# HilaManor/AudioEditingCode

Measured on AMD Instinct MI355X. Metric: edited-clips/sec (200-step inv+edit, 10 s@16 kHz), higher is better.
Workload: dtype f32

## Files before the change

### audioeditingcode_amd/csrc/attention.hip

```cpp
#include <mutex>
#include "aed_common.h"

typedef float f32x4 __attribute__((ext_vector_type(4)));

#include "attn_params.h"

#define KV_TILE 64
#define Q_TILE 64

template <int D>
__global__ __launch_bounds__(256) void attention_kernel(AttnParams p) {
    constexpr int KLD = D + 4;
    constexpr int VLD = KV_TILE + 4;
    constexpr int NB = D / 16;
    __shared__ __attribute__((aligned(16))) float Ks[KV_TILE * KLD];
    __shared__ __attribute__((aligned(16))) float Vt[D * VLD];
    __shared__ __attribute__((aligned(16))) float Ps[4 * 16 * VLD];

    const int tid = threadIdx.x;
    const int lane = tid & 63, wave = tid >> 6;
    const int fi = lane & 15, fh = lane >> 4;
    const int b = blockIdx.z, head = blockIdx.y;
    const int q0 = blockIdx.x * Q_TILE + wave * 16;
    const int hoff = head * D;

    const float* Q = p.q + (size_t)b * p.bsq + hoff;
    const float* K = p.k + (size_t)b * p.bsk + hoff;
    const float* V = p.v + (size_t)b * p.bsv + hoff;
    const float* bias = p.bias ? p.bias + (size_t)b * p.ld_bias : nullptr;

    float4 qf[NB];
    {
        const int qr = q0 + fi;
#pragma unroll
        for (int blk = 0; blk < NB; ++blk) {
            qf[blk] = make_float4(0.f, 0.f, 0.f, 0.f);
            if (qr < p.Nq) qf[blk] = *reinterpret_cast<const float4*>(Q + (size_t)qr * p.ldq + 16 * blk + 4 * fh);
        }
    }
    f32x4 oacc[NB];
#pragma unroll
    for (int c = 0; c < NB; ++c) oacc[c] = (f32x4){0.f, 0.f, 0.f, 0.f};
    float m_run[4], l_run[4];
#pragma unroll
    for (int r = 0; r < 4; ++r) { m_run[r] = -INFINITY; l_run[r] = 0.f; }

    float* Pw = Ps + wave * 16 * VLD;

    for (int k0 = 0; k0 < p.Nk; k0 += KV_TILE) {
        for (int idx = tid; idx < KV_TILE * (D / 4); idx += 256) {
            const int key = idx / (D / 4), c4 = idx - key * (D / 4);
            float4 v = make_float4(0.f, 0.f, 0.f, 0.f);
            if (k0 + key < p.Nk) v = *reinterpret_cast<const float4*>(K + (size_t)(k0 + key) * p.ldk + 4 * c4);
            *reinterpret_cast<float4*>(Ks + key * KLD + 4 * c4) = v;
        }
        {
            const int key = tid & 63, dg = tid >> 6;
            for (int dd = dg * 4; dd < D; dd += 16) {
                float4 v = make_float4(0.f, 0.f, 0.f, 0.f);
                if (k0 + key < p.Nk) v = *reinterpret_cast<const float4*>(V + (size_t)(k0 + key) * p.ldv + dd);
                Vt[(dd + 0) * VLD + key] = v.x;
                Vt[(dd + 1) * VLD + key] = v.y;
                Vt[(dd + 2) * VLD + key] = v.z;
                Vt[(dd + 3) * VLD + key] = v.w;
            }
        }
        __syncthreads();

        f32x4 sacc[4];
#pragma unroll
        for (int j = 0; j < 4; ++j) sacc[j] = (f32x4){0.f, 0.f, 0.f, 0.f};
#pragma unroll
        for (int blk = 0; blk < NB; ++blk) {
#pragma unroll
            for (int j = 0; j < 4; ++j) {
                const float4 kf = *reinterpret_cast<const float4*>(Ks + (16 * j + fi) * KLD + 16 * blk + 4 * fh);
                sacc[j] = __builtin_amdgcn_mfma_f32_16x16x4f32(qf[blk].x, kf.x, sacc[j], 0, 0, 0);
                sacc[j] = __builtin_amdgcn_mfma_f32_16x16x4f32(qf[blk].y, kf.y, sacc[j], 0, 0, 0);
                sacc[j] = __builtin_amdgcn_mfma_f32_16x16x4f32(qf[blk].z, kf.z, sacc[j], 0, 0, 0);
                sacc[j] = __builtin_amdgcn_mfma_f32_16x16x4f32(qf[blk].w, kf.w, sacc[j], 0, 0, 0);
            }
        }
        float tmax[4];
#pragma unroll
        for (int r = 0; r < 4; ++r) tmax[r] = -INFINITY;
#pragma unroll
        for (int j = 0; j < 4; ++j) {
            const int key = k0 + 16 * j + fi;
            const bool ok = key < p.Nk;
            const float bv = (ok && bias) ? bias[key] : 0.f;
#pragma unroll
            for (int r = 0; r < 4; ++r) {
                float s = ok ? sacc[j][r] * p.scale + bv : -INFINITY;
                sacc[j][r] = s;
                tmax[r] = fmaxf(tmax[r], s);
            }
        }
#pragma unroll
        for (int r = 0; r < 4; ++r) {
#pragma unroll
            for (int o = 8; o > 0; o >>= 1) tmax[r] = fmaxf(tmax[r], __shfl_xor(tmax[r], o, 16));
        }
        float alpha[4], rsum[4];
#pragma unroll
        for (int r = 0; r < 4; ++r) {
            const float mn = fmaxf(m_run[r], tmax[r]);
            alpha[r] = __expf(m_run[r] - mn);
            m_run[r] = mn;
            rsum[r] = 0.f;
        }
#pragma unroll
        for (int j = 0; j < 4; ++j) {
#pragma unroll
            for (int r = 0; r < 4; ++r) {
                const float pv = __expf(sacc[j][r] - m_run[r]);
                rsum[r] += pv;
                Pw[(4 * fh + r) * VLD + 16 * j + fi] = pv;
            }
        }
#pragma unroll
        for (int r = 0; r < 4; ++r) {
#pragma unroll
            for (int o = 8; o > 0; o >>= 1) rsum[r] += __shfl_xor(rsum[r], o, 16);
            l_run[r] = l_run[r] * alpha[r] + rsum[r];
        }
#pragma unroll
        for (int c = 0; c < NB; ++c)
#pragma unroll
            for (int r = 0; r < 4; ++r) oacc[c][r] *= alpha[r];

        __builtin_amdgcn_fence(__ATOMIC_ACQ_REL, "wavefront");
        __builtin_amdgcn_wave_barrier();

#pragma unroll
        for (int kb = 0; kb < 4; ++kb) {
            const float4 pf = *reinterpret_cast<const float4*>(Pw + fi * VLD + 16 * kb + 4 * fh);
#pragma unroll
            for (int c = 0; c < NB; ++c) {
                const float4 vf = *reinterpret_cast<const float4*>(Vt + (16 * c + fi) * VLD + 16 * kb + 4 * fh);
                oacc[c] = __builtin_amdgcn_mfma_f32_16x16x4f32(pf.x, vf.x, oacc[c], 0, 0, 0);
                oacc[c] = __builtin_amdgcn_mfma_f32_16x16x4f32(pf.y, vf.y, oacc[c], 0, 0, 0);
                oacc[c] = __builtin_amdgcn_mfma_f32_16x16x4f32(pf.z, vf.z, oacc[c], 0, 0, 0);
                oacc[c] = __builtin_amdgcn_mfma_f32_16x16x4f32(pf.w, vf.w, oacc[c], 0, 0, 0);
            }
        }
        __syncthreads();
    }

    float* O = p.o + (size_t)b * p.bso + hoff;
#pragma unroll
    for (int r = 0; r < 4; ++r) {
        const int qr = q0 + 4 * fh + r;
        if (qr >= p.Nq) continue;
        const float inv = 1.0f / l_run[r];
#pragma unroll
        for (int c = 0; c < NB; ++c) O[(size_t)qr * p.ldo + 16 * c + fi] = oacc[c][r] * inv;
    }
}

typedef float f32x16a __attribute__((ext_vector_type(16)));

template <int D, int KSPLIT>
__global__ __launch_bounds__(256) void attention_t_kernel(AttnParams p) {
    constexpr int DT = (D + 31) / 32;
    constexpr int KLD = D + 4;
    constexpr int VLD = 32 + 4;
    constexpr int NJ = D / 8;
    constexpr int SLAB = 32 * KLD + DT * 32 * VLD;
    constexpr int MSZ = DT * 16 + 2;
    static_assert(D % 8 == 0, "head dim");
    extern __shared__ __attribute__((aligned(16))) float smem[];
    const int tid = threadIdx.x, lane = tid & 63, wave = tid >> 6;
    const int fi = lane & 31, fh = lane >> 5;
    float* Ks = smem + wave * SLAB;
    float* Vt = Ks + 32 * KLD;

    int qt, head, b;
    {
        const unsigned nx = gridDim.x, ny = gridDim.y, nwg = nx * ny * gridDim.z;
        const unsigned orig = blockIdx.x + nx * (blockIdx.y + ny * blockIdx.z);
        const unsigned xcd = orig & 7u, q = nwg >> 3, r = nwg & 7u;
        const unsigned id = (xcd < r ? xcd * (q + 1) : r * (q + 1) + (xcd - r) * q) + (orig >> 3);
        qt = (int)(id % nx);
        head = (int)((id / nx) % ny);
        b = (int)(id / (nx * ny));
    }
    const int q0 = (KSPLIT == 1 ? qt * 128 + wave * 32 : qt * 32);
    const int hoff = head * D;
    const float* Q = p.q + (size_t)b * p.bsq + hoff;
    const float* K = p.k + (size_t)b * p.bsk + hoff;
    const float* V = p.v + (size_t)b * p.bsv + hoff;
    const float* bias = p.bias ? p.bias + (size_t)b * p.ld_bias : nullptr;

    float4 qf[NJ];
    {
        const int qr = min(q0 + fi, p.Nq - 1);
#pragma unroll
        for (int j = 0; j < NJ; ++j) {
            float4 v = *reinterpret_cast<const float4*>(Q + (size_t)qr * p.ldq + 8 * j + 4 * fh);
            qf[j] = make_float4(v.x * p.scale, v.y * p.scale, v.z * p.scale, v.w * p.scale);
        }
    }
    f32x16a oacc[DT];
#pragma unroll
    for (int c = 0; c < DT; ++c)
#pragma unroll
        for (int r = 0; r < 16; ++r) oacc[c][r] = 0.f;
    float m_run = -INFINITY, l_run = 0.f;

    constexpr int KC4 = D / 4;
    constexpr int NKL = (32 * KC4) / 64;
    float4 kreg[NKL], vreg[NKL];
    const int ntiles = (p.Nk + 31) / 32;
    auto prefetch = [&](int t) {
        const int k0 = min(t, ntiles - 1) * 32;
#pragma unroll
        for (int i = 0; i < NKL; ++i) {
            const int idx = lane + 64 * i;
            const int key = min(k0 + idx / KC4, p.Nk - 1);
            kreg[i] = *reinterpret_cast<const float4*>(K + (size_t)key * p.ldk + 4 * (idx % KC4));
        }
        const int vk = min(k0 + fi, p.Nk - 1);
#pragma unroll
        for (int i = 0; i < NKL; ++i)
            vreg[i] = *reinterpret_cast<const float4*>(V + (size_t)vk * p.ldv + 4 * (2 * i + fh));
    };
    auto stage = [&]() {
#pragma unroll
        for (int i = 0; i < NKL; ++i) {
            const int idx = lane + 64 * i;
            const float4 v = kreg[i];
            *reinterpret_cast<float4*>(Ks + (idx / KC4) * KLD + 4 * (idx % KC4)) = make_float4(v.x, v.y, v.z, v.w);
        }
#pragma unroll
        for (int i = 0; i < NKL; ++i) {
            const int dd = 4 * (2 * i + fh);
            const float4 v = vreg[i];
            Vt[(dd + 0) * VLD + fi] = v.x;
            Vt[(dd + 1) * VLD + fi] = v.y;
            Vt[(dd + 2) * VLD + fi] = v.z;
            Vt[(dd + 3) * VLD + fi] = v.w;
        }
    };
    if constexpr (DT * 32 > D) {
        for (int e = lane; e < (DT * 32 - D) * VLD; e += 64) Vt[D * VLD + e] = 0.f;
    }

    const int t_first = (KSPLIT == 1 ? 0 : wave);
    constexpr int TSTEP = (KSPLIT == 1 ? 1 : KSPLIT);
    prefetch(t_first);
    for (int t = t_first; t < ntiles; t += TSTEP) {
        stage();
        prefetch(t + TSTEP);
        asm volatile("" ::: "memory");
        __builtin_amdgcn_wave_barrier();
        f32x16a sacc;
#pragma unroll
        for (int r = 0; r < 16; ++r) sacc[r] = 0.f;
#pragma unroll
        for (int j = 0; j < NJ; ++j) {
            const float4 kf = *reinterpret_cast<const float4*>(Ks + fi * KLD + 8 * j + 4 * fh);
            sacc = __builtin_amdgcn_mfma_f32_32x32x2f32(kf.x, qf[j].x, sacc, 0, 0, 0);
            sacc = __builtin_amdgcn_mfma_f32_32x32x2f32(kf.y, qf[j].y, sacc, 0, 0, 0);
            sacc = __builtin_amdgcn_mfma_f32_32x32x2f32(kf.z, qf[j].z, sacc, 0, 0, 0);
            sacc = __builtin_amdgcn_mfma_f32_32x32x2f32(kf.w, qf[j].w, sacc, 0, 0, 0);
        }
        const int k0 = t * 32;
        if (bias) {
#pragma unroll
            for (int rq = 0; rq < 4; ++rq)
#pragma unroll
                for (int e = 0; e < 4; ++e)
                    sacc[4 * rq + e] += bias[min(k0 + 8 * rq + 4 * fh + e, p.Nk - 1)];
        }
        if (k0 + 32 > p.Nk) {
#pragma unroll
            for (int r = 0; r < 16; ++r)
                if (k0 + (r & 3) + 8 * (r >> 2) + 4 * fh >= p.Nk) sacc[r] = -INFINITY;
        }
        float mx = sacc[0];
#pragma unroll
        for (int r = 1; r < 16; ++r) mx = fmaxf(mx, sacc[r]);
        {
            auto sw = __builtin_amdgcn_permlane32_swap(__float_as_uint(mx), __float_as_uint(mx), false, false);
            mx = fmaxf(__uint_as_float(sw[0]), __uint_as_float(sw[1]));
        }
        const float mn = fmaxf(m_run, mx);
        const float alpha = __expf(m_run - mn);
        m_run = mn;
        float rsum = 0.f;
#pragma unroll
        for (int r = 0; r < 16; ++r) {
            sacc[r] = __expf(sacc[r] - mn);
            rsum += sacc[r];
        }
        l_run = l_run * alpha + rsum;
#pragma unroll
        for (int c = 0; c < DT; ++c)
#pragma unroll
            for (int r = 0; r < 16; ++r) oacc[c][r] *= alpha;
#pragma unroll
        for (int rq = 0; rq < 4; ++rq) {
#pragma unroll
            for (int c = 0; c < DT; ++c) {
                const float4 vf = *reinterpret_cast<const float4*>(Vt + (c * 32 + fi) * VLD + 8 * rq + 4 * fh);
                oacc[c] = __builtin_amdgcn_mfma_f32_32x32x2f32(vf.x, sacc[4 * rq + 0], oacc[c], 0, 0, 0);
                oacc[c] = __builtin_amdgcn_mfma_f32_32x32x2f32(vf.y, sacc[4 * rq + 1], oacc[c], 0, 0, 0);
                oacc[c] = __builtin_amdgcn_mfma_f32_32x32x2f32(vf.z, sacc[4 * rq + 2], oacc[c], 0, 0, 0);
                oacc[c] = __builtin_amdgcn_mfma_f32_32x32x2f32(vf.w, sacc[4 * rq + 3], oacc[c], 0, 0, 0);
            }
        }
        asm volatile("" ::: "memory");
        __builtin_amdgcn_wave_barrier();
    }

    if constexpr (KSPLIT > 1) {
        __syncthreads();
        float* mrg = smem;
        if (wave > 0) {
            float* dst = mrg + ((wave - 1) * 64 + lane) * MSZ;
            dst[0] = m_run;
            dst[1] = l_run;
#pragma unroll
            for (int c = 0; c < DT; ++c)
#pragma unroll
                for (int r = 0; r < 16; ++r) dst[2 + 16 * c + r] = oacc[c][r];
        }
        __syncthreads();
        if (wave > 0) return;
        float mt = m_run;
#pragma unroll
        for (int w = 0; w < KSPLIT - 1; ++w) mt = fmaxf(mt, mrg[(w * 64 + lane) * MSZ]);
        const float a0 = (m_run == -INFINITY) ? 0.f : __expf(m_run - mt);
        l_run *= a0;
#pragma unroll
        for (int c = 0; c < DT; ++c)
#pragma unroll
            for (int r = 0; r < 16; ++r) oacc[c][r] *= a0;
#pragma unroll
        for (int w = 0; w < KSPLIT - 1; ++w) {
            const float* src = mrg + (w * 64 + lane) * MSZ;
            const float mw = src[0];
            const float aw = (mw == -INFINITY) ? 0.f : __expf(mw - mt);
            l_run += src[1] * aw;
#pragma unroll
            for (int c = 0; c < DT; ++c)
#pragma unroll
                for (int r = 0; r < 16; ++r) oacc[c][r] += src[2 + 16 * c + r] * aw;
        }
    }
    {
        auto sw = __builtin_amdgcn_permlane32_swap(__float_as_uint(l_run), __float_as_uint(l_run), false, false);
        l_run = __uint_as_float(sw[0]) + __uint_as_float(sw[1]);
    }
    const float inv = 1.0f / l_run;
    const int qr = q0 + fi;
    if (qr < p.Nq) {
        float* O = p.o + (size_t)b * p.bso + hoff + (size_t)qr * p.ldo;
#pragma unroll
        for (int c = 0; c < DT; ++c)
#pragma unroll
            for (int rq = 0; rq < 4; ++rq) {
                const int d0 = c * 32 + 8 * rq + 4 * fh;
                if (d0 < D)
                    *reinterpret_cast<float4*>(O + d0) = make_float4(oacc[c][4 * rq] * inv, oacc[c][4 * rq + 1] * inv,
                                                                     oacc[c][4 * rq + 2] * inv, oacc[c][4 * rq + 3] * inv);
            }
    }
}

template <int D, int KSPLIT>
static int launch_t(const AttnParams& p, int B, hipStream_t s) {
    constexpr int DT = (D + 31) / 32;
    constexpr int SLAB = 32 * (D + 4) + DT * 32 * 36;
    constexpr int MRG = (KSPLIT - 1) * 64 * (DT * 16 + 2);
    const size_t bytes = sizeof(float) * (4 * SLAB > MRG ? 4 * SLAB : MRG);
    static std::once_flag attr_once;
    static hipError_t attr_rc = hipSuccess;
    std::call_once(attr_once, [&] {
        attr_rc = hipFuncSetAttribute((const void*)attention_t_kernel<D, KSPLIT>,
                                      hipFuncAttributeMaxDynamicSharedMemorySize, (int)bytes);
    });
    AED_CHECK_HIP(attr_rc);
    dim3 grid(aed_cdiv(p.Nq, KSPLIT == 1 ? 128 : 32), p.H, B);
    hipLaunchKernelGGL((attention_t_kernel<D, KSPLIT>), grid, dim3(256), bytes, s, p);
    return 0;
}

int launch_attention(const aed_op* op, hipStream_t s) {
    const int32_t* i = op->i;
    AttnParams p;
    p.q = (const float*)op->p[0]; p.k = (const float*)op->p[1]; p.v = (const float*)op->p[2];
    p.bias = (const float*)op->p[3]; p.o = (float*)op->p[4];
    AED_REQUIRE(p.q && p.k && p.v && p.o, "attention: null pointer");
    p.H = i[1]; p.Nq = i[2]; p.Nk = i[3];
    p.ldq = i[5]; p.ldk = i[6]; p.ldv = i[7]; p.ldo = i[8]; p.ld_bias = i[9];
    p.bsq = i[10]; p.bsk = i[11]; p.bsv = i[12]; p.bso = i[13];
    p.scale = op->f[0];
    AED_REQUIRE(p.ldq % 4 == 0 && p.ldk % 4 == 0 && p.ldv % 4 == 0, "attention: row strides must be multiples of 4");
    AED_REQUIRE(p.Nq > 0 && p.Nk > 0, "attention: empty sequence");
    AED_REQUIRE(p.ldo % 4 == 0, "attention: output row stride must be a multiple of 4");
    if (p.Nk > KV_TILE && i[14] != 1) {
        const long wg_ksplit1 = (long)aed_cdiv(p.Nq, 128) * p.H * i[0];
        const bool ks4 = wg_ksplit1 < 2L * aed_num_cus();
        int rc = 0;
        if (((op->flags & 4) && !ks4) || i[14] == 3) {
            rc = launch_attention_x6(p, i[0], i[4], s);
            if (rc >= 0) return rc;
            AED_REQUIRE(i[14] != 3, "attention: the split-bf16 kernel does not take head dim %d / these operands", i[4]);
        }
        switch (i[4]) {
            case 32: rc = ks4 ? launch_t<32, 4>(p, i[0], s) : launch_t<32, 1>(p, i[0], s); break;
            case 48: rc = ks4 ? launch_t<48, 4>(p, i[0], s) : launch_t<48, 1>(p, i[0], s); break;
            case 64: rc = ks4 ? launch_t<64, 4>(p, i[0], s) : launch_t<64, 1>(p, i[0], s); break;
            case 80: rc = ks4 ? launch_t<80, 4>(p, i[0], s) : launch_t<80, 1>(p, i[0], s); break;
            case 16: rc = ks4 ? launch_t<16, 4>(p, i[0], s) : launch_t<16, 1>(p, i[0], s); break;
            default: AED_REQUIRE(false, "attention: unsupported head dim %d (16/32/48/64/80)", i[4]);
        }
        if (rc) return rc;
        AED_CHECK_HIP(hipGetLastError());
        return 0;
    }
    dim3 grid(aed_cdiv(p.Nq, Q_TILE), p.H, i[0]);
    switch (i[4]) {
        case 16: hipLaunchKernelGGL(attention_kernel<16>, grid, dim3(256), 0, s, p); break;
        case 32: hipLaunchKernelGGL(attention_kernel<32>, grid, dim3(256), 0, s, p); break;
        case 48: hipLaunchKernelGGL(attention_kernel<48>, grid, dim3(256), 0, s, p); break;
        case 64: hipLaunchKernelGGL(attention_kernel<64>, grid, dim3(256), 0, s, p); break;
        case 80: hipLaunchKernelGGL(attention_kernel<80>, grid, dim3(256), 0, s, p); break;
        default: AED_REQUIRE(false, "attention: unsupported head dim %d (16/32/48/64/80)", i[4]);
    }
    AED_CHECK_HIP(hipGetLastError());
    return 0;
}
```

### audioeditingcode_amd/csrc/attention_x6.hip

```cpp
#include "attn_params.h"

typedef __bf16 abf16x8 __attribute__((ext_vector_type(8)));
typedef __bf16 abf16x2 __attribute__((ext_vector_type(2)));
typedef float af32x2 __attribute__((ext_vector_type(2)));
typedef float af32x16 __attribute__((ext_vector_type(16)));

__device__ __forceinline__ void ax6_split_pair(float x0, float x1, unsigned& h, unsigned& m, unsigned& l) {
    h = __builtin_bit_cast(unsigned, __builtin_convertvector((af32x2){x0, x1}, abf16x2));
    float r0 = x0 - __uint_as_float(h << 16);
    float r1 = x1 - __uint_as_float(h & 0xffff0000u);
    asm volatile("" : "+v"(r0), "+v"(r1));
    m = __builtin_bit_cast(unsigned, __builtin_convertvector((af32x2){r0, r1}, abf16x2));
    float q0 = r0 - __uint_as_float(m << 16);
    float q1 = r1 - __uint_as_float(m & 0xffff0000u);
    asm volatile("" : "+v"(q0), "+v"(q1));
    l = __builtin_bit_cast(unsigned, __builtin_convertvector((af32x2){q0, q1}, abf16x2));
}

__device__ __forceinline__ void ax6_split8(const float (&x)[8], abf16x8 (&f)[3]) {
    uint4 h, m, l;
    ax6_split_pair(x[0], x[1], h.x, m.x, l.x);
    ax6_split_pair(x[2], x[3], h.y, m.y, l.y);
    ax6_split_pair(x[4], x[5], h.z, m.z, l.z);
    ax6_split_pair(x[6], x[7], h.w, m.w, l.w);
    f[0] = __builtin_bit_cast(abf16x8, h);
    f[1] = __builtin_bit_cast(abf16x8, m);
    f[2] = __builtin_bit_cast(abf16x8, l);
}

__device__ __forceinline__ void ax6_mfma6(af32x16& acc, const abf16x8 (&a)[3], const abf16x8 (&b)[3]) {
    acc = __builtin_amdgcn_mfma_f32_32x32x16_bf16(a[0], b[2], acc, 0, 0, 0);
    acc = __builtin_amdgcn_mfma_f32_32x32x16_bf16(a[2], b[0], acc, 0, 0, 0);
    acc = __builtin_amdgcn_mfma_f32_32x32x16_bf16(a[1], b[1], acc, 0, 0, 0);
    acc = __builtin_amdgcn_mfma_f32_32x32x16_bf16(a[0], b[1], acc, 0, 0, 0);
    acc = __builtin_amdgcn_mfma_f32_32x32x16_bf16(a[1], b[0], acc, 0, 0, 0);
    acc = __builtin_amdgcn_mfma_f32_32x32x16_bf16(a[0], b[0], acc, 0, 0, 0);
}

template <int D>
__global__ __launch_bounds__(256, 2) void attention_x6_kernel(AttnParams p) {
    constexpr int NDB = D / 16;
    constexpr int DT = (D + 31) / 32;
    constexpr int KQ = NDB * 3 * 64;
    constexpr int VQ = 2 * 3 * DT * 64;
    constexpr int STAGE = KQ + VQ;
    constexpr int C4 = D / 4;
    constexpr int NK = (8 * D + 255) / 256;
    constexpr int NV = (8 * D + 255) / 256;
    static_assert(D % 16 == 0 && 2 * STAGE * 16 <= 65536, "head dim");
    __shared__ uint4 lds[2 * STAGE];

    const int tid = threadIdx.x, lane = tid & 63, wave = tid >> 6;
    const int fi = lane & 31, fh = lane >> 5;
    int qt, head, b;
    {
        const unsigned nx = gridDim.x, ny = gridDim.y, nwg = nx * ny * gridDim.z;
        const unsigned orig = blockIdx.x + nx * (blockIdx.y + ny * blockIdx.z);
        const unsigned xcd = orig & 7u, q = nwg >> 3, r = nwg & 7u;
        const unsigned id = (xcd < r ? xcd * (q + 1) : r * (q + 1) + (xcd - r) * q) + (orig >> 3);
        qt = (int)(id % nx);
        head = (int)((id / nx) % ny);
        b = (int)(id / (nx * ny));
    }
    const int q0 = qt * 128 + wave * 32;
    const int hoff = head * D;
    const float* Q = p.q + (size_t)b * p.bsq + hoff;
    const float* K = p.k + (size_t)b * p.bsk + hoff;
    const float* V = p.v + (size_t)b * p.bsv + hoff;
    const float* bias = p.bias ? p.bias + (size_t)b * p.ld_bias : nullptr;

    abf16x8 qp[NDB][3];
    {
        const float* qrow = Q + (size_t)min(q0 + fi, p.Nq - 1) * p.ldq + 8 * fh;
#pragma unroll
        for (int db = 0; db < NDB; ++db) {
            const float4 a = *reinterpret_cast<const float4*>(qrow + 16 * db);
            const float4 c = *reinterpret_cast<const float4*>(qrow + 16 * db + 4);
            const float x[8] = {a.x * p.scale, a.y * p.scale, a.z * p.scale, a.w * p.scale,
                                c.x * p.scale, c.y * p.scale, c.z * p.scale, c.w * p.scale};
            ax6_split8(x, qp[db]);
        }
    }
    af32x16 oacc[DT];
#pragma unroll
    for (int c = 0; c < DT; ++c)
#pragma unroll
        for (int r = 0; r < 16; ++r) oacc[c][r] = 0.f;
    float m_run = -INFINITY, l_run = 0.f;

    const int ntiles = (p.Nk + 31) / 32;
    float4 kreg[2][NK];
    float vreg[2][NV][4];
    auto prefetch = [&](int t, float4 (&kr)[NK], float (&vr)[NV][4]) {
        const int k0 = min(t, ntiles - 1) * 32;
#pragma unroll
        for (int i = 0; i < NK; ++i) {
            const int item = min(tid + 256 * i, 8 * D - 1);
            const int key = min(k0 + item / C4, p.Nk - 1);
            kr[i] = *reinterpret_cast<const float4*>(K + (size_t)key * p.ldk + 4 * (item % C4));
        }
#pragma unroll
        for (int i = 0; i < NV; ++i) {
            const int item = min(tid + 256 * i, 8 * D - 1);
            const int kg = item / D, d = item - kg * D;
#pragma unroll
            for (int j = 0; j < 4; ++j)
                vr[i][j] = V[(size_t)min(k0 + 4 * kg + j, p.Nk - 1) * p.ldv + d];
        }
    };
    auto stage_write = [&](uint4* st, const float4 (&kr)[NK], const float (&vr)[NV][4]) {
        uint2* k2 = reinterpret_cast<uint2*>(st);
        uint2* v2 = reinterpret_cast<uint2*>(st + KQ);
#pragma unroll
        for (int i = 0; i < NK; ++i) {
            const int item = tid + 256 * i;
            if (8 * D % 256 != 0 && item >= 8 * D) break;
            const int key = item / C4, c4 = item % C4;
            unsigned h0, m0, l0, h1, m1, l1;
            ax6_split_pair(kr[i].x, kr[i].y, h0, m0, l0);
            ax6_split_pair(kr[i].z, kr[i].w, h1, m1, l1);
            uint2* dst = k2 + ((c4 >> 2) * 3 * 32 + key) * 4 + ((c4 >> 1) & 1) * 2 + (c4 & 1);
            dst[0] = make_uint2(h0, h1);
            dst[32 * 4] = make_uint2(m0, m1);
            dst[2 * 32 * 4] = make_uint2(l0, l1);
        }
#pragma unroll
        for (int i = 0; i < NV; ++i) {
            const int item = tid + 256 * i;
            if (8 * D % 256 != 0 && item >= 8 * D) break;
            const int kg = item / D, d = item - kg * D;
            unsigned h0, m0, l0, h1, m1, l1;
            ax6_split_pair(vr[i][0], vr[i][1], h0, m0, l0);
            ax6_split_pair(vr[i][2], vr[i][3], h1, m1, l1);
            const int kb = kg >> 2, g = kg & 3;
            uint2* dst = v2 + (((kb * 3) * DT + (d >> 5)) * 32 + (d & 31)) * 4 + (g & 1) * 2 + (g >> 1);
            dst[0] = make_uint2(h0, h1);
            dst[DT * 32 * 4] = make_uint2(m0, m1);
            dst[2 * DT * 32 * 4] = make_uint2(l0, l1);
        }
    };
    if constexpr (DT * 32 > D) {
        for (int e = tid; e < 2 * STAGE; e += 256) lds[e] = make_uint4(0u, 0u, 0u, 0u);
        __syncthreads();
    }

    prefetch(0, kreg[0], vreg[0]);
    prefetch(1, kreg[1], vreg[1]);
    stage_write(lds, kreg[0], vreg[0]);
    prefetch(2, kreg[0], vreg[0]);
    __syncthreads();
    for (int t0 = 0; t0 < ntiles; t0 += 2) {
#pragma unroll
        for (int u = 0; u < 2; ++u) {
            const int t = t0 + u;
            const uint4* st = lds + u * STAGE;
            af32x16 sacc;
#pragma unroll
            for (int r = 0; r < 16; ++r) sacc[r] = 0.f;
#pragma unroll
            for (int db = 0; db < NDB; ++db) {
                abf16x8 kf[3];
#pragma unroll
                for (int pl = 0; pl < 3; ++pl) kf[pl] = __builtin_bit_cast(abf16x8, st[((db * 3 + pl) * 32 + fi) * 2 + fh]);
                ax6_mfma6(sacc, kf, qp[db]);
            }
            stage_write(lds + (u ^ 1) * STAGE, kreg[u ^ 1], vreg[u ^ 1]);
            prefetch(t + 3, kreg[u ^ 1], vreg[u ^ 1]);
            const int k0 = t * 32;
            if (bias) {
#pragma unroll
                for (int rq = 0; rq < 4; ++rq)
#pragma unroll
                    for (int e = 0; e < 4; ++e)
                        sacc[4 * rq + e] += bias[min(k0 + 8 * rq + 4 * fh + e, p.Nk - 1)];
            }
            if (k0 + 32 > p.Nk) {
#pragma unroll
                for (int r = 0; r < 16; ++r)
                    if (k0 + (r & 3) + 8 * (r >> 2) + 4 * fh >= p.Nk) sacc[r] = -INFINITY;
            }
            float mx = sacc[0];
#pragma unroll
            for (int r = 1; r < 16; ++r) mx = fmaxf(mx, sacc[r]);
            {
                auto sw = __builtin_amdgcn_permlane32_swap(__float_as_uint(mx), __float_as_uint(mx), false, false);
                mx = fmaxf(__uint_as_float(sw[0]), __uint_as_float(sw[1]));
            }
            const float mn = fmaxf(m_run, mx);
            const float alpha = __expf(m_run - mn);
            m_run = mn;
            float rsum = 0.f;
#pragma unroll
            for (int r = 0; r < 16; ++r) {
                sacc[r] = __expf(sacc[r] - mn);
                rsum += sacc[r];
            }
            l_run = l_run * alpha + rsum;
#pragma unroll
            for (int c = 0; c < DT; ++c)
#pragma unroll
                for (int r = 0; r < 16; ++r) oacc[c][r] *= alpha;
#pragma unroll
            for (int kb = 0; kb < 2; ++kb) {
                abf16x8 pf[3];
                const float x[8] = {sacc[8 * kb], sacc[8 * kb + 1], sacc[8 * kb + 2], sacc[8 * kb + 3],
                                    sacc[8 * kb + 4], sacc[8 * kb + 5], sacc[8 * kb + 6], sacc[8 * kb + 7]};
                ax6_split8(x, pf);
#pragma unroll
                for (int c = 0; c < DT; ++c) {
                    abf16x8 vf[3];
#pragma unroll
                    for (int pl = 0; pl < 3; ++pl)
                        vf[pl] = __builtin_bit_cast(abf16x8, st[KQ + (((kb * 3 + pl) * DT + c) * 32 + fi) * 2 + fh]);
                    ax6_mfma6(oacc[c], vf, pf);
                }
            }
            __syncthreads();
        }
    }

    {
        auto sw = __builtin_amdgcn_permlane32_swap(__float_as_uint(l_run), __float_as_uint(l_run), false, false);
        l_run = __uint_as_float(sw[0]) + __uint_as_float(sw[1]);
    }
    const float inv = 1.0f / l_run;
    const int qr = q0 + fi;
    if (qr < p.Nq) {
        float* O = p.o + (size_t)b * p.bso + hoff + (size_t)qr * p.ldo;
#pragma unroll
        for (int c = 0; c < DT; ++c)
#pragma unroll
            for (int rq = 0; rq < 4; ++rq) {
                const int d0 = c * 32 + 8 * rq + 4 * fh;
                if (d0 < D)
                    *reinterpret_cast<float4*>(O + d0) = make_float4(oacc[c][4 * rq] * inv, oacc[c][4 * rq + 1] * inv,
                                                                     oacc[c][4 * rq + 2] * inv, oacc[c][4 * rq + 3] * inv);
            }
    }
}

template <int D>
static int launch_ax6(const AttnParams& p, int B, hipStream_t s) {
    dim3 grid(aed_cdiv(p.Nq, 128), p.H, B);
    hipLaunchKernelGGL((attention_x6_kernel<D>), grid, dim3(256), 0, s, p);
    AED_CHECK_HIP(hipGetLastError());
    return 0;
}

int launch_attention_x6(const AttnParams& p, int B, int D, hipStream_t s) {
    if (((uintptr_t)p.q | (uintptr_t)p.k) % 16 != 0) return -1;
    switch (D) {
        case 32: return launch_ax6<32>(p, B, s);
        case 48: return launch_ax6<48>(p, B, s);
        case 64: return launch_ax6<64>(p, B, s);
        default: return -1;
    }
}
```

### audioeditingcode_amd/csrc/attn_params.h

```cpp
#pragma once
#include "aed_common.h"

struct AttnParams {
    const float* q; const float* k; const float* v; const float* bias; float* o;
    int Nq, Nk, H;
    int ldq, ldk, ldv, ldo, ld_bias;
    long bsq, bsk, bsv, bso;
    float scale;
};

int launch_attention_x6(const AttnParams& p, int B, int D, hipStream_t s);
```

Measured before the change: 0.9055.

## Rewrite split-bf16 attention kernel with register prefetch and buffer loads

Adds a new split-bf16 MFMA attention kernel that prefetches K/V tiles into registers two stages ahead via buffer loads with bounds clamping. It splits the data into bf16 planes while writing to double-buffered LDS, and interleaves the next tile's staging with the current tile's compute. Full tiles run without masking and only the tail is masked. The old kernel is kept as a reference path, chosen by a new forcing flag or when the offsets could overflow 32 bits. The aim is to hide global load latency and cut barrier and masking overhead, at the cost of more registers and more code complexity.

```diff
diff --git a/audioeditingcode_amd/csrc/attention.hip b/audioeditingcode_amd/csrc/attention.hip
--- a/audioeditingcode_amd/csrc/attention.hip
+++ b/audioeditingcode_amd/csrc/attention.hip
@@ -400,14 +400,15 @@
     AED_REQUIRE(p.ldq % 4 == 0 && p.ldk % 4 == 0 && p.ldv % 4 == 0, "attention: row strides must be multiples of 4");
     AED_REQUIRE(p.Nq > 0 && p.Nk > 0, "attention: empty sequence");
     AED_REQUIRE(p.ldo % 4 == 0, "attention: output row stride must be a multiple of 4");
-    if (p.Nk > KV_TILE && i[14] != 1) {
+    const bool forced = i[14] == 3 || i[14] == 4;
+    if ((p.Nk > KV_TILE && i[14] != 1) || forced) {
         const long wg_ksplit1 = (long)aed_cdiv(p.Nq, 128) * p.H * i[0];
         const bool ks4 = wg_ksplit1 < 2L * aed_num_cus();
         int rc = 0;
-        if (((op->flags & 4) && !ks4) || i[14] == 3) {
-            rc = launch_attention_x6(p, i[0], i[4], s);
+        if (((op->flags & 4) && !ks4) || forced) {
+            rc = launch_attention_x6(p, i[0], i[4], i[14] == 4, s);
             if (rc >= 0) return rc;
-            AED_REQUIRE(i[14] != 3, "attention: the split-bf16 kernel does not take head dim %d / these operands", i[4]);
+            AED_REQUIRE(!forced, "attention: the split-bf16 kernel does not take head dim %d / these operands", i[4]);
         }
         switch (i[4]) {
             case 32: rc = ks4 ? launch_t<32, 4>(p, i[0], s) : launch_t<32, 1>(p, i[0], s); break;
diff --git a/audioeditingcode_amd/csrc/attention_x6.hip b/audioeditingcode_amd/csrc/attention_x6.hip
--- a/audioeditingcode_amd/csrc/attention_x6.hip
+++ b/audioeditingcode_amd/csrc/attention_x6.hip
@@ -37,8 +37,242 @@
     acc = __builtin_amdgcn_mfma_f32_32x32x16_bf16(a[0], b[0], acc, 0, 0, 0);
 }
 
+typedef float af32x4 __attribute__((ext_vector_type(4)));
+template <int V> struct ax6_c { static constexpr int value = V; };
+
 template <int D>
 __global__ __launch_bounds__(256, 2) void attention_x6_kernel(AttnParams p) {
+    constexpr int NT = 256;
+    constexpr int NDB = D / 16;
+    constexpr int DT = (D + 31) / 32;
+    constexpr int KQ = NDB * 3 * 64;
+    constexpr int VQ = 2 * 3 * DT * 64;
+    constexpr int STAGE = KQ + VQ;
+    constexpr int C4 = D / 4;
+    constexpr int NI = (16 * D + NT - 1) / NT;
+    static_assert(D % 16 == 0 && 2 * STAGE * 16 <= 65536, "head dim");
+    __shared__ uint4 lds[2 * STAGE];
+
+    const int tid = threadIdx.x, lane = tid & 63;
+    const int wave = __builtin_amdgcn_readfirstlane(tid >> 6);
+    const int fi = lane & 31, fh = lane >> 5;
+    int qt, head, b;
+    {
+        const unsigned nx = gridDim.x, ny = gridDim.y, nwg = nx * ny * gridDim.z;
+        const unsigned orig = blockIdx.x + nx * (blockIdx.y + ny * blockIdx.z);
+        const unsigned xcd = orig & 7u, q = nwg >> 3, r = nwg & 7u;
+        const unsigned id = (xcd < r ? xcd * (q + 1) : r * (q + 1) + (xcd - r) * q) + (orig >> 3);
+        qt = (int)(id % nx);
+        head = (int)((id / nx) % ny);
+        b = (int)(id / (nx * ny));
+    }
+    const int q0 = qt * 128 + wave * 32;
+    const int hoff = head * D;
+    const float* Q = p.q + (size_t)b * p.bsq + hoff;
+
+    abf16x8 qp[NDB][3];
+    {
+        const float* qrow = Q + (size_t)min(q0 + fi, p.Nq - 1) * p.ldq + 8 * fh;
+#pragma unroll
+        for (int db = 0; db < NDB; ++db) {
+            const float4 a = *reinterpret_cast<const float4*>(qrow + 16 * db);
+            const float4 c = *reinterpret_cast<const float4*>(qrow + 16 * db + 4);
+            const float x[8] = {a.x * p.scale, a.y * p.scale, a.z * p.scale, a.w * p.scale,
+                                c.x * p.scale, c.y * p.scale, c.z * p.scale, c.w * p.scale};
+            ax6_split8(x, qp[db]);
+        }
+    }
+    af32x16 oacc[DT];
+#pragma unroll
+    for (int c = 0; c < DT; ++c)
+#pragma unroll
+        for (int r = 0; r < 16; ++r) oacc[c][r] = 0.f;
+    float m_run = -INFINITY, l_run = 0.f;
+
+    const int ntiles = (p.Nk + 31) / 32;
+    auto is_k = [&](int i) { return NT * (i + 1) <= 8 * D ? true : NT * i >= 8 * D ? false : wave * 64 + NT * i < 8 * D; };
+    auto is_v = [&](int i) {
+        return NT * (i + 1) <= 8 * D ? false : (NT * i >= 8 * D && NT * (i + 1) <= 16 * D) ? true
+                                             : (wave * 64 + NT * i >= 8 * D && wave * 64 + NT * i < 16 * D);
+    };
+    unsigned off[NI][4];
+#pragma unroll
+    for (int i = 0; i < NI; ++i) {
+        const int item = tid + NT * i;
+        if (is_k(i)) {
+            off[i][0] = 4u * (unsigned)((item / C4) * p.ldk + 4 * (item % C4));
+            off[i][1] = off[i][2] = off[i][3] = 0u;
+        } else {
+            const int it = item - 8 * D, kg = it / D, d = it - kg * D;
+#pragma unroll
+            for (int j = 0; j < 4; ++j) off[i][j] = 4u * (unsigned)((4 * kg + j) * p.ldv + d);
+        }
+    }
+    const char* kbase = reinterpret_cast<const char*>(p.k + (size_t)b * p.bsk + hoff);
+    const char* vbase = reinterpret_cast<const char*>(p.v + (size_t)b * p.bsv + hoff);
+    const int kstep = 128 * p.ldk, vstep = 128 * p.ldv;
+    int krem = 4 * ((p.Nk - 1) * p.ldk + D), vrem = 4 * ((p.Nk - 1) * p.ldv + D);
+    const __amdgpu_buffer_rsrc_t srd_b = __builtin_amdgcn_make_buffer_rsrc(
+        (void*)(p.bias ? p.bias + (size_t)b * p.ld_bias : p.k), 0, p.bias ? 4 * p.Nk : 0, 0x00020000);
+
+    af32x4 reg[2][NI];
+    auto prefetch = [&](af32x4 (&rg)[NI]) {
+        const __amdgpu_buffer_rsrc_t srd_k = __builtin_amdgcn_make_buffer_rsrc((void*)kbase, 0, krem, 0x00020000);
+        const __amdgpu_buffer_rsrc_t srd_v = __builtin_amdgcn_make_buffer_rsrc((void*)vbase, 0, vrem, 0x00020000);
+#pragma unroll
+        for (int i = 0; i < NI; ++i) {
+            if (is_k(i)) {
+                rg[i] = __builtin_bit_cast(af32x4, __builtin_amdgcn_raw_buffer_load_b128(srd_k, off[i][0], 0, 0));
+            } else if (is_v(i)) {
+#pragma unroll
+                for (int j = 0; j < 4; ++j)
+                    rg[i][j] = __uint_as_float(__builtin_amdgcn_raw_buffer_load_b32(srd_v, off[i][j], 0, 0));
+            }
+        }
+        kbase += kstep; krem = max(krem - kstep, 0);
+        vbase += vstep; vrem = max(vrem - vstep, 0);
+    };
+    auto stage_write = [&](uint4* st, const af32x4 (&rg)[NI]) {
+        uint2* k2 = reinterpret_cast<uint2*>(st);
+        uint2* v2 = reinterpret_cast<uint2*>(st + KQ);
+#pragma unroll
+        for (int i = 0; i < NI; ++i) {
+            const int item = tid + NT * i;
+            unsigned h0, m0, l0, h1, m1, l1;
+            if (is_k(i)) {
+                const int key = item / C4, c4 = item % C4;
+                ax6_split_pair(rg[i][0], rg[i][1], h0, m0, l0);
+                ax6_split_pair(rg[i][2], rg[i][3], h1, m1, l1);
+                uint2* dst = k2 + ((c4 >> 2) * 3 * 32 + key) * 4 + ((c4 >> 1) & 1) * 2 + (c4 & 1);
+                dst[0] = make_uint2(h0, h1);
+                dst[32 * 4] = make_uint2(m0, m1);
+                dst[2 * 32 * 4] = make_uint2(l0, l1);
+            } else if (is_v(i)) {
+                const int it = item - 8 * D, kg = it / D, d = it - kg * D;
+                ax6_split_pair(rg[i][0], rg[i][1], h0, m0, l0);
+                ax6_split_pair(rg[i][2], rg[i][3], h1, m1, l1);
+                const int kb = kg >> 2, g = kg & 3;
+                uint2* dst = v2 + (((kb * 3) * DT + (d >> 5)) * 32 + (d & 31)) * 4 + (g & 1) * 2 + (g >> 1);
+                dst[0] = make_uint2(h0, h1);
+                dst[DT * 32 * 4] = make_uint2(m0, m1);
+                dst[2 * DT * 32 * 4] = make_uint2(l0, l1);
+            }
+        }
+    };
+    if constexpr (DT * 32 > D) {
+        for (int e = tid; e < 2 * STAGE; e += NT) lds[e] = make_uint4(0u, 0u, 0u, 0u);
+        __syncthreads();
+    }
+
+    auto tile = [&](auto uc, auto mc, const int t) {
+        constexpr int u = decltype(uc)::value;
+        constexpr bool MASKED = decltype(mc)::value != 0;
+        const uint4* st = lds + u * STAGE;
+        af32x16 sacc;
+#pragma unroll
+        for (int r = 0; r < 16; ++r) sacc[r] = 0.f;
+#pragma unroll
+        for (int db = 0; db < NDB; ++db) {
+            abf16x8 kf[3];
+#pragma unroll
+            for (int pl = 0; pl < 3; ++pl) kf[pl] = __builtin_bit_cast(abf16x8, st[((db * 3 + pl) * 32 + fi) * 2 + fh]);
+            ax6_mfma6(sacc, kf, qp[db]);
+        }
+        stage_write(lds + (u ^ 1) * STAGE, reg[u ^ 1]);
+        prefetch(reg[u ^ 1]);
+        const int k0 = t * 32;
+        if (p.bias) {
+            const unsigned bo = 4u * (unsigned)(k0 + 4 * fh);
+#pragma unroll
+            for (int rq = 0; rq < 4; ++rq)
+#pragma unroll
+                for (int e = 0; e < 4; ++e)
+                    sacc[4 * rq + e] += __uint_as_float(__builtin_amdgcn_raw_buffer_load_b32(srd_b, bo + 4u * (8 * rq + e), 0, 0));
+        }
+        if constexpr (MASKED) {
+            if (k0 + 32 > p.Nk) {
+#pragma unroll
+                for (int r = 0; r < 16; ++r)
+                    if (k0 + (r & 3) + 8 * (r >> 2) + 4 * fh >= p.Nk) sacc[r] = -INFINITY;
+            }
+        }
+        float mx = sacc[0];
+#pragma unroll
+        for (int r = 1; r < 16; ++r) mx = fmaxf(mx, sacc[r]);
+        {
+            auto sw = __builtin_amdgcn_permlane32_swap(__float_as_uint(mx), __float_as_uint(mx), false, false);
+            mx = fmaxf(__uint_as_float(sw[0]), __uint_as_float(sw[1]));
+        }
+        const float mn = fmaxf(m_run, mx);
+        const float alpha = __expf(m_run - mn);
+        m_run = mn;
+        float rsum = 0.f;
+#pragma unroll
+        for (int r = 0; r < 16; ++r) {
+            sacc[r] = __expf(sacc[r] - mn);
+            rsum += sacc[r];
+        }
+        l_run = l_run * alpha + rsum;
+#pragma unroll
+        for (int c = 0; c < DT; ++c)
+#pragma unroll
+            for (int r = 0; r < 16; ++r) oacc[c][r] *= alpha;
+#pragma unroll
+        for (int kb = 0; kb < 2; ++kb) {
+            abf16x8 pf[3];
+            const float x[8] = {sacc[8 * kb], sacc[8 * kb + 1], sacc[8 * kb + 2], sacc[8 * kb + 3],
+                                sacc[8 * kb + 4], sacc[8 * kb + 5], sacc[8 * kb + 6], sacc[8 * kb + 7]};
+            ax6_split8(x, pf);
+#pragma unroll
+            for (int c = 0; c < DT; ++c) {
+                abf16x8 vf[3];
+#pragma unroll
+                for (int pl = 0; pl < 3; ++pl)
+                    vf[pl] = __builtin_bit_cast(abf16x8, st[KQ + (((kb * 3 + pl) * DT + c) * 32 + fi) * 2 + fh]);
+                ax6_mfma6(oacc[c], vf, pf);
+            }
+        }
+        __syncthreads();
+    };
+
+    prefetch(reg[0]);
+    prefetch(reg[1]);
+    stage_write(lds, reg[0]);
+    prefetch(reg[0]);
+    __syncthreads();
+    const int nmain = (p.Nk / 32) & ~1;
+    int t0 = 0;
+    for (; t0 < nmain; t0 += 2) {
+        tile(ax6_c<0>{}, ax6_c<0>{}, t0);
+        tile(ax6_c<1>{}, ax6_c<0>{}, t0 + 1);
+    }
+    if (t0 < ntiles) {
+        tile(ax6_c<0>{}, ax6_c<1>{}, t0);
+        tile(ax6_c<1>{}, ax6_c<1>{}, t0 + 1);
+    }
+
+    {
+        auto sw = __builtin_amdgcn_permlane32_swap(__float_as_uint(l_run), __float_as_uint(l_run), false, false);
+        l_run = __uint_as_float(sw[0]) + __uint_as_float(sw[1]);
+    }
+    const float inv = 1.0f / l_run;
+    const int qr = q0 + fi;
+    if (qr < p.Nq) {
+        float* O = p.o + (size_t)b * p.bso + hoff + (size_t)qr * p.ldo;
+#pragma unroll
+        for (int c = 0; c < DT; ++c)
+#pragma unroll
+            for (int rq = 0; rq < 4; ++rq) {
+                const int d0 = c * 32 + 8 * rq + 4 * fh;
+                if (d0 < D)
+                    *reinterpret_cast<float4*>(O + d0) = make_float4(oacc[c][4 * rq] * inv, oacc[c][4 * rq + 1] * inv,
+                                                                     oacc[c][4 * rq + 2] * inv, oacc[c][4 * rq + 3] * inv);
+            }
+    }
+}
+
+template <int D>
+__global__ __launch_bounds__(256, 2) void attention_x6_ref_kernel(AttnParams p) {
     constexpr int NDB = D / 16;
     constexpr int DT = (D + 31) / 32;
     constexpr int KQ = NDB * 3 * 64;
@@ -240,19 +474,29 @@
 }
 
 template <int D>
-static int launch_ax6(const AttnParams& p, int B, hipStream_t s) {
+static int launch_ax6_ref(const AttnParams& p, int B, hipStream_t s) {
+    dim3 grid(aed_cdiv(p.Nq, 128), p.H, B);
+    hipLaunchKernelGGL((attention_x6_ref_kernel<D>), grid, dim3(256), 0, s, p);
+    AED_CHECK_HIP(hipGetLastError());
+    return 0;
+}
+
+template <int D>
+static int launch_ax6(const AttnParams& p, int B, bool reference, hipStream_t s) {
+    const bool fits = ((long)p.Nk + 96) * (p.ldk > p.ldv ? p.ldk : p.ldv) * 4 < (1L << 31);
+    if (reference || !fits) return launch_ax6_ref<D>(p, B, s);
     dim3 grid(aed_cdiv(p.Nq, 128), p.H, B);
     hipLaunchKernelGGL((attention_x6_kernel<D>), grid, dim3(256), 0, s, p);
     AED_CHECK_HIP(hipGetLastError());
     return 0;
 }
 
-int launch_attention_x6(const AttnParams& p, int B, int D, hipStream_t s) {
+int launch_attention_x6(const AttnParams& p, int B, int D, bool reference, hipStream_t s) {
     if (((uintptr_t)p.q | (uintptr_t)p.k) % 16 != 0) return -1;
     switch (D) {
-        case 32: return launch_ax6<32>(p, B, s);
-        case 48: return launch_ax6<48>(p, B, s);
-        case 64: return launch_ax6<64>(p, B, s);
+        case 32: return launch_ax6<32>(p, B, reference, s);
+        case 48: return launch_ax6<48>(p, B, reference, s);
+        case 64: return launch_ax6<64>(p, B, reference, s);
         default: return -1;
     }
 }
diff --git a/audioeditingcode_amd/csrc/attn_params.h b/audioeditingcode_amd/csrc/attn_params.h
--- a/audioeditingcode_amd/csrc/attn_params.h
+++ b/audioeditingcode_amd/csrc/attn_params.h
@@ -9,4 +9,4 @@
     float scale;
 };
 
-int launch_attention_x6(const AttnParams& p, int B, int D, hipStream_t s);
+int launch_attention_x6(const AttnParams& p, int B, int D, bool reference, hipStream_t s);
```

After: 0.9573 (median of 6 runs). 1.06x the previous value.
